# skyplane-project/skyplane

Measured on NVIDIA H100. Metric: chunk-pipeline GB/s (raw input), higher is better.
Workload: dtype u8/u32

## Files before the change

skyplane_b200/csrc/md5.cuh:

```cuda
#pragma once
#include <stdint.h>

#include <type_traits>
#include <utility>

#ifndef SKY_MD5_SLOTS
#define SKY_MD5_SLOTS 4
#endif

namespace sky {

struct Md5State {
    uint32_t a, b, c, d;
};

__device__ __forceinline__ void md5_init(Md5State &s) {
    s.a = 0x67452301u;
    s.b = 0xefcdab89u;
    s.c = 0x98badcfeu;
    s.d = 0x10325476u;
}

__device__ __forceinline__ uint32_t md5_am(uint32_t a, uint32_t m, uint32_t one) {
    uint32_t r;
    asm("mad.lo.u32 %0, %1, %2, %3;" : "=r"(r) : "r"(m), "r"(one), "r"(a));
    return r;
}
__device__ __forceinline__ uint32_t md5_one() {
    uint32_t eq, lane;
    asm("mov.u32 %0, %%lanemask_eq;" : "=r"(eq));
    asm("mov.u32 %0, %%laneid;" : "=r"(lane));
    return eq >> lane;
}
#define SKY_MD5_STEP(FN, a, b, c, d, m, k, s)                      \
    {                                                              \
        uint32_t t_ = FN(b, c, d) + md5_am(a, (m), one) + (k);     \
        a = b + __funnelshift_l(t_, t_, s);                        \
    }
#define SKY_F(b, c, d) ((d) ^ ((b) & ((c) ^ (d))))
#define SKY_G(b, c, d) ((c) ^ ((d) & ((b) ^ (c))))
#define SKY_H(b, c, d) ((b) ^ (c) ^ (d))
#define SKY_I(b, c, d) ((c) ^ ((b) | ~(d)))

template <int R>
__device__ __forceinline__ void md5_round(uint32_t &a, uint32_t &b, uint32_t &c, uint32_t &d, const uint32_t (&w)[16],
                                          uint32_t one) {
    if constexpr (R == 0) {
        SKY_MD5_STEP(SKY_F, a, b, c, d, w[0], 0xd76aa478, 7)
        SKY_MD5_STEP(SKY_F, d, a, b, c, w[1], 0xe8c7b756, 12)
        SKY_MD5_STEP(SKY_F, c, d, a, b, w[2], 0x242070db, 17)
        SKY_MD5_STEP(SKY_F, b, c, d, a, w[3], 0xc1bdceee, 22)
        SKY_MD5_STEP(SKY_F, a, b, c, d, w[4], 0xf57c0faf, 7)
        SKY_MD5_STEP(SKY_F, d, a, b, c, w[5], 0x4787c62a, 12)
        SKY_MD5_STEP(SKY_F, c, d, a, b, w[6], 0xa8304613, 17)
        SKY_MD5_STEP(SKY_F, b, c, d, a, w[7], 0xfd469501, 22)
        SKY_MD5_STEP(SKY_F, a, b, c, d, w[8], 0x698098d8, 7)
        SKY_MD5_STEP(SKY_F, d, a, b, c, w[9], 0x8b44f7af, 12)
        SKY_MD5_STEP(SKY_F, c, d, a, b, w[10], 0xffff5bb1, 17)
        SKY_MD5_STEP(SKY_F, b, c, d, a, w[11], 0x895cd7be, 22)
        SKY_MD5_STEP(SKY_F, a, b, c, d, w[12], 0x6b901122, 7)
        SKY_MD5_STEP(SKY_F, d, a, b, c, w[13], 0xfd987193, 12)
        SKY_MD5_STEP(SKY_F, c, d, a, b, w[14], 0xa679438e, 17)
        SKY_MD5_STEP(SKY_F, b, c, d, a, w[15], 0x49b40821, 22)
    } else if constexpr (R == 1) {
        SKY_MD5_STEP(SKY_G, a, b, c, d, w[1], 0xf61e2562, 5)
        SKY_MD5_STEP(SKY_G, d, a, b, c, w[6], 0xc040b340, 9)
        SKY_MD5_STEP(SKY_G, c, d, a, b, w[11], 0x265e5a51, 14)
        SKY_MD5_STEP(SKY_G, b, c, d, a, w[0], 0xe9b6c7aa, 20)
        SKY_MD5_STEP(SKY_G, a, b, c, d, w[5], 0xd62f105d, 5)
        SKY_MD5_STEP(SKY_G, d, a, b, c, w[10], 0x02441453, 9)
        SKY_MD5_STEP(SKY_G, c, d, a, b, w[15], 0xd8a1e681, 14)
        SKY_MD5_STEP(SKY_G, b, c, d, a, w[4], 0xe7d3fbc8, 20)
        SKY_MD5_STEP(SKY_G, a, b, c, d, w[9], 0x21e1cde6, 5)
        SKY_MD5_STEP(SKY_G, d, a, b, c, w[14], 0xc33707d6, 9)
        SKY_MD5_STEP(SKY_G, c, d, a, b, w[3], 0xf4d50d87, 14)
        SKY_MD5_STEP(SKY_G, b, c, d, a, w[8], 0x455a14ed, 20)
        SKY_MD5_STEP(SKY_G, a, b, c, d, w[13], 0xa9e3e905, 5)
        SKY_MD5_STEP(SKY_G, d, a, b, c, w[2], 0xfcefa3f8, 9)
        SKY_MD5_STEP(SKY_G, c, d, a, b, w[7], 0x676f02d9, 14)
        SKY_MD5_STEP(SKY_G, b, c, d, a, w[12], 0x8d2a4c8a, 20)
    } else if constexpr (R == 2) {
        SKY_MD5_STEP(SKY_H, a, b, c, d, w[5], 0xfffa3942, 4)
        SKY_MD5_STEP(SKY_H, d, a, b, c, w[8], 0x8771f681, 11)
        SKY_MD5_STEP(SKY_H, c, d, a, b, w[11], 0x6d9d6122, 16)
        SKY_MD5_STEP(SKY_H, b, c, d, a, w[14], 0xfde5380c, 23)
        SKY_MD5_STEP(SKY_H, a, b, c, d, w[1], 0xa4beea44, 4)
        SKY_MD5_STEP(SKY_H, d, a, b, c, w[4], 0x4bdecfa9, 11)
        SKY_MD5_STEP(SKY_H, c, d, a, b, w[7], 0xf6bb4b60, 16)
        SKY_MD5_STEP(SKY_H, b, c, d, a, w[10], 0xbebfbc70, 23)
        SKY_MD5_STEP(SKY_H, a, b, c, d, w[13], 0x289b7ec6, 4)
        SKY_MD5_STEP(SKY_H, d, a, b, c, w[0], 0xeaa127fa, 11)
        SKY_MD5_STEP(SKY_H, c, d, a, b, w[3], 0xd4ef3085, 16)
        SKY_MD5_STEP(SKY_H, b, c, d, a, w[6], 0x04881d05, 23)
        SKY_MD5_STEP(SKY_H, a, b, c, d, w[9], 0xd9d4d039, 4)
        SKY_MD5_STEP(SKY_H, d, a, b, c, w[12], 0xe6db99e5, 11)
        SKY_MD5_STEP(SKY_H, c, d, a, b, w[15], 0x1fa27cf8, 16)
        SKY_MD5_STEP(SKY_H, b, c, d, a, w[2], 0xc4ac5665, 23)
    } else {
        SKY_MD5_STEP(SKY_I, a, b, c, d, w[0], 0xf4292244, 6)
        SKY_MD5_STEP(SKY_I, d, a, b, c, w[7], 0x432aff97, 10)
        SKY_MD5_STEP(SKY_I, c, d, a, b, w[14], 0xab9423a7, 15)
        SKY_MD5_STEP(SKY_I, b, c, d, a, w[5], 0xfc93a039, 21)
        SKY_MD5_STEP(SKY_I, a, b, c, d, w[12], 0x655b59c3, 6)
        SKY_MD5_STEP(SKY_I, d, a, b, c, w[3], 0x8f0ccc92, 10)
        SKY_MD5_STEP(SKY_I, c, d, a, b, w[10], 0xffeff47d, 15)
        SKY_MD5_STEP(SKY_I, b, c, d, a, w[1], 0x85845dd1, 21)
        SKY_MD5_STEP(SKY_I, a, b, c, d, w[8], 0x6fa87e4f, 6)
        SKY_MD5_STEP(SKY_I, d, a, b, c, w[15], 0xfe2ce6e0, 10)
        SKY_MD5_STEP(SKY_I, c, d, a, b, w[6], 0xa3014314, 15)
        SKY_MD5_STEP(SKY_I, b, c, d, a, w[13], 0x4e0811a1, 21)
        SKY_MD5_STEP(SKY_I, a, b, c, d, w[4], 0xf7537e82, 6)
        SKY_MD5_STEP(SKY_I, d, a, b, c, w[11], 0xbd3af235, 10)
        SKY_MD5_STEP(SKY_I, c, d, a, b, w[2], 0x2ad7d2bb, 15)
        SKY_MD5_STEP(SKY_I, b, c, d, a, w[9], 0xeb86d391, 21)
    }
}

__device__ __forceinline__ void md5_block(Md5State &st, const uint32_t (&w)[16], uint32_t one) {
    uint32_t a = st.a, b = st.b, c = st.c, d = st.d;
    md5_round<0>(a, b, c, d, w, one);
    md5_round<1>(a, b, c, d, w, one);
    md5_round<2>(a, b, c, d, w, one);
    md5_round<3>(a, b, c, d, w, one);
    st.a += a;
    st.b += b;
    st.c += c;
    st.d += d;
}

template <int kSlot>
__device__ __forceinline__ void cp_async_block(bool pred, uint32_t lane_ring, const uint8_t *gptr) {
    asm volatile(
        "{\n\t.reg .pred p;\n\t"
        "setp.ne.b32 p, %2, 0;\n\t"
        "@p cp.async.cg.shared.global [%0+%3], [%1], 16;\n\t"
        "@p cp.async.cg.shared.global [%0+%4], [%1+16], 16;\n\t"
        "@p cp.async.cg.shared.global [%0+%5], [%1+32], 16;\n\t"
        "@p cp.async.cg.shared.global [%0+%6], [%1+48], 16;\n\t}" ::"r"(lane_ring),
        "l"(gptr), "r"((uint32_t)pred), "n"(kSlot * 2048), "n"(kSlot * 2048 + 512), "n"(kSlot * 2048 + 1024),
        "n"(kSlot * 2048 + 1536)
        : "memory");
}
__device__ __forceinline__ void cp_async_commit() { asm volatile("cp.async.commit_group;\n" ::: "memory"); }
template <int N>
__device__ __forceinline__ void cp_async_wait() {
    asm volatile("cp.async.wait_group %0;\n" ::"n"(N) : "memory");
}

template <class F, int... I>
__device__ __forceinline__ void md5_unroll_(F &&f, std::integer_sequence<int, I...>) {
    (f(std::integral_constant<int, I>()), ...);
}
template <int N, class F>
__device__ __forceinline__ void md5_unroll(F &&f) {
    md5_unroll_(f, std::make_integer_sequence<int, N>());
}

struct Md5NoGate {
    __device__ __forceinline__ void operator()(uint64_t, bool) const {}
};

template <class Gate = Md5NoGate>
__device__ __forceinline__ void md5_warp(uint32_t *ring, const uint8_t *src, uint64_t len, bool active, uint8_t *out,
                                         unsigned lane, Gate gate = Gate()) {
    constexpr int kSlots = SKY_MD5_SLOTS;
    static_assert(kSlots >= 2 && (kSlots & (kSlots - 1)) == 0 && 1024 % kSlots == 0, "SKY_MD5_SLOTS: a power of two, 2..1024");
    constexpr bool kGated = !std::is_same<Gate, Md5NoGate>::value;
    const uint32_t nfull = active ? (uint32_t)(len >> 6) : 0;
    const uint32_t wmax = __reduce_max_sync(0xffffffffu, nfull);
    const uint32_t trips = (wmax + (kSlots - 1)) & ~(uint32_t)(kSlots - 1);
    Md5State st;
    md5_init(st);
    Md5State fin = st;
    const uint32_t *lring = ring + lane * 4;
    const uint32_t lring_s = (uint32_t)__cvta_generic_to_shared(lring);
    const uint32_t one = md5_one();

    gate(0, active && len > 0);
    md5_unroll<kSlots - 1>([&](auto sc) {
        constexpr int s = decltype(sc)::value;
        cp_async_block<s>((uint32_t)s < nfull, lring_s, src + s * 64);
        cp_async_commit();
    });
    auto load_words = [&](uint32_t (&w)[16], int cs) {
#pragma unroll
        for (int q = 0; q < 4; q++) {
            const uint4 v = *reinterpret_cast<const uint4 *>(lring + (cs * 4 + q) * 128);
            w[4 * q + 0] = v.x;
            w[4 * q + 1] = v.y;
            w[4 * q + 2] = v.z;
            w[4 * q + 3] = v.w;
        }
    };
    uint32_t w[2][16];
    cp_async_wait<kSlots - 2>();
    load_words(w[0], 0);
    const uint8_t *pf_src = src + (kSlots - 1) * 64;
    auto blocks = [&](uint32_t i) {
        md5_unroll<kSlots>([&](auto uc) {
            constexpr int u = decltype(uc)::value;
            constexpr int ps = (u + kSlots - 1) & (kSlots - 1);
            constexpr int ns = (u + 1) & (kSlots - 1);
            uint32_t a = st.a, b = st.b, c = st.c, d = st.d;
            md5_round<0>(a, b, c, d, w[u & 1], one);
            cp_async_block<ps>(i + u + (kSlots - 1) < nfull, lring_s, pf_src + u * 64);
            md5_round<1>(a, b, c, d, w[u & 1], one);
            cp_async_commit();
            cp_async_wait<kSlots - 2>();
            md5_round<2>(a, b, c, d, w[u & 1], one);
            load_words(w[(u + 1) & 1], ns);
            md5_round<3>(a, b, c, d, w[u & 1], one);
            st.a += a;
            st.b += b;
            st.c += c;
            st.d += d;
            if (i + u < nfull) fin = st;
        });
        pf_src += kSlots * 64;
    };
    if constexpr (kGated) {
        for (uint32_t base = 0; base < trips; base += 1024) {
            gate((base >> 10) + 1, (uint64_t)(base + 1024) * 64 < len);
            const uint32_t iend = min(base + 1024, trips);
            for (uint32_t i = base; i < iend; i += kSlots) blocks(i);
        }
    } else {
        for (uint32_t i = 0; i < trips; i += kSlots) blocks(i);
    }
    cp_async_wait<0>();
    st = fin;
    if (active) {
        const uint32_t rem = (uint32_t)(len & 63);
        const uint8_t *tp = src + ((uint64_t)nfull << 6);
        uint32_t tw[32];
#pragma unroll
        for (int k = 0; k < 32; k++) tw[k] = 0;
        for (uint32_t k = 0; k < rem; k++) tw[k >> 2] |= (uint32_t)tp[k] << (8 * (k & 3));
        tw[rem >> 2] |= 0x80u << (8 * (rem & 3));
        const bool two = rem >= 56;
        const uint64_t bits = len << 3;
        tw[two ? 30 : 14] = (uint32_t)bits;
        tw[two ? 31 : 15] = (uint32_t)(bits >> 32);
        for (int t = 0; t < (two ? 2 : 1); t++) {
            uint32_t w[16];
#pragma unroll
            for (int k = 0; k < 16; k++) w[k] = tw[16 * t + k];
            md5_block(st, w, one);
        }
        uint4 dg = make_uint4(st.a, st.b, st.c, st.d);
        *reinterpret_cast<uint4 *>(out) = dg;
    }
}

}
```

skyplane_b200/native.py:

```python
from __future__ import annotations

import ctypes
from pathlib import Path
from typing import Optional, Sequence

_PKG = Path(__file__).resolve().parent
LIB_PATH = _PKG / "libskychunk.so"

SKY_OK = 0
SKY_E_INVALID, SKY_E_NOGPU, SKY_E_CUDA, SKY_E_CAPACITY, SKY_E_BUSY, SKY_E_TICKET, SKY_E_NOMEM, SKY_E_NOKEY = -1, -2, -3, -4, -5, -6, -7, -8
F_LZ4, F_MD5, F_E2EE, F_HC = 1, 2, 16, 32
BOX_OVERHEAD = 40
D_OK, D_BAD_HEADER, D_CORRUPT, D_SIZE, D_UNSUPPORTED, D_LAYOUT, D_TRUNCATED, D_AUTH = 0, -1, -2, -3, -4, -5, -6, -7
D_NAMES = {0: "ok", -1: "bad frame header", -2: "corrupt block", -3: "size mismatch", -4: "unsupported frame feature",
           -5: "unexpected block layout", -6: "truncated frame", -7: "box authentication failed"}

ABI_SYMBOLS = (
    "sky_strerror", "sky_last_error", "sky_abi_version", "sky_device_count", "sky_device_pci_bus_id", "sky_kernel_config", "sky_frame_bound",
    "sky_ctx_create", "sky_ctx_destroy", "sky_pinned_alloc", "sky_pinned_free",
    "sky_submit", "sky_wait", "sky_set_e2ee_key", "sky_box_bound", "sky_process_device", "sky_decode_device", "sky_decode",
    "sky_device_alloc", "sky_device_free", "sky_memcpy_h2d", "sky_memcpy_d2h", "sky_launch_count",
)


class SkyChunkError(RuntimeError):
    def __init__(self, code: int, detail: str = ""):
        self.code = code
        msg = f"libskychunk error {code}: {_strerror(code)}"
        if detail:
            msg += f" [{detail}]"
        super().__init__(msg)


_lib: Optional[ctypes.CDLL] = None


def _strerror(code: int) -> str:
    try:
        return lib().sky_strerror(code).decode()
    except Exception:
        return "?"


def lib() -> ctypes.CDLL:
    global _lib
    if _lib is not None:
        return _lib
    import os

    from skyplane_b200 import build as _build

    override = os.environ.get("SKYCHUNK_LIB")
    if override:
        L = ctypes.CDLL(override)
    else:
        if _build.needs_build():
            _build.build()
        L = ctypes.CDLL(str(LIB_PATH))
    vp, u64, u32, i32 = ctypes.c_void_p, ctypes.c_uint64, ctypes.c_uint32, ctypes.c_int
    p_u64 = ctypes.POINTER(u64)
    L.sky_strerror.argtypes = [i32]
    L.sky_strerror.restype = ctypes.c_char_p
    L.sky_last_error.argtypes = [vp]
    L.sky_last_error.restype = ctypes.c_char_p
    L.sky_abi_version.argtypes = []
    L.sky_abi_version.restype = i32
    L.sky_device_count.argtypes = [ctypes.POINTER(i32)]
    L.sky_device_count.restype = i32
    L.sky_device_pci_bus_id.argtypes = [i32, ctypes.c_char_p, i32]
    L.sky_device_pci_bus_id.restype = i32
    L.sky_kernel_config.argtypes = [i32]
    L.sky_kernel_config.restype = u32
    L.sky_frame_bound.argtypes = [u64]
    L.sky_frame_bound.restype = u64
    L.sky_ctx_create.argtypes = [i32, u64, u32, u32, ctypes.POINTER(vp)]
    L.sky_ctx_create.restype = i32
    L.sky_ctx_destroy.argtypes = [vp]
    L.sky_ctx_destroy.restype = i32
    L.sky_pinned_alloc.argtypes = [u64]
    L.sky_pinned_alloc.restype = vp
    L.sky_pinned_free.argtypes = [vp]
    L.sky_pinned_free.restype = i32
    L.sky_submit.argtypes = [vp, u32, ctypes.POINTER(vp), p_u64, ctypes.POINTER(vp), p_u64, u32, ctypes.c_char_p, p_u64]
    L.sky_submit.restype = i32
    L.sky_set_e2ee_key.argtypes = [vp, ctypes.c_char_p]
    L.sky_set_e2ee_key.restype = i32
    L.sky_box_bound.argtypes = [u64]
    L.sky_box_bound.restype = u64
    L.sky_wait.argtypes = [vp, u64, p_u64, vp, ctypes.POINTER(ctypes.c_float)]
    L.sky_wait.restype = i32
    L.sky_process_device.argtypes = [vp, u32, vp, p_u64, p_u64, vp, p_u64, p_u64, u32, vp, p_u64, vp, ctypes.POINTER(ctypes.c_float)]
    L.sky_process_device.restype = i32
    p_i32 = ctypes.POINTER(ctypes.c_int32)
    L.sky_decode_device.argtypes = [vp, u32, vp, p_u64, p_u64, vp, p_u64, p_u64, vp, p_i32, vp, ctypes.POINTER(ctypes.c_float)]
    L.sky_decode_device.restype = i32
    L.sky_decode.argtypes = [vp, u32, ctypes.POINTER(vp), p_u64, ctypes.POINTER(vp), p_u64, u32, p_i32, vp, ctypes.POINTER(ctypes.c_float)]
    L.sky_decode.restype = i32
    L.sky_device_alloc.argtypes = [vp, u64, ctypes.POINTER(vp)]
    L.sky_device_alloc.restype = i32
    L.sky_device_free.argtypes = [vp, vp]
    L.sky_device_free.restype = i32
    L.sky_memcpy_h2d.argtypes = [vp, vp, vp, u64]
    L.sky_memcpy_h2d.restype = i32
    L.sky_memcpy_d2h.argtypes = [vp, vp, vp, u64]
    L.sky_memcpy_d2h.restype = i32
    L.sky_launch_count.argtypes = [vp]
    L.sky_launch_count.restype = u64
    _lib = L
    return L


def device_pci_bus_id(device: int) -> str:
    buf = ctypes.create_string_buffer(32)
    rc = lib().sky_device_pci_bus_id(device, buf, 32)
    if rc != SKY_OK:
        raise SkyChunkError(rc)
    return buf.value.decode().lower()


def kernel_config() -> dict:
    L = lib()
    return {"lz4_entries": L.sky_kernel_config(0), "warps": L.sky_kernel_config(1), "seg_slots": L.sky_kernel_config(2),
            "max_step_log": L.sky_kernel_config(3), "hc_depth": L.sky_kernel_config(4), "hc_hash_bits": L.sky_kernel_config(5),
            "hc_nice": L.sky_kernel_config(6)}


def frame_bound(n: int) -> int:
    return int(lib().sky_frame_bound(n))


def round16(x: int) -> int:
    return (x + 15) & ~15


def device_count() -> int:
    n = ctypes.c_int(0)
    rc = lib().sky_device_count(ctypes.byref(n))
    if rc != SKY_OK:
        return 0
    return n.value


class PinnedBuffer:

    def __init__(self, nbytes: int):
        self.nbytes = int(nbytes)
        self.addr = lib().sky_pinned_alloc(self.nbytes)
        if not self.addr:
            raise SkyChunkError(SKY_E_NOMEM, "sky_pinned_alloc failed (no CUDA device?)")
        self._arr = (ctypes.c_ubyte * max(1, self.nbytes)).from_address(self.addr)
        self.view = memoryview(self._arr).cast("B")[: self.nbytes]

    def close(self):
        if self.addr:
            self.view.release()
            del self._arr
            lib().sky_pinned_free(self.addr)
            self.addr = None

    def __del__(self):
        try:
            self.close()
        except Exception:
            pass


class Context:

    def __init__(self, device: int = 0, max_batch_bytes: int = 1 << 30, max_chunks: int = 1024, n_slots: int = 2):
        self._h = ctypes.c_void_p()
        self.device = device
        self.max_chunks = max_chunks
        self.max_batch_bytes = max_batch_bytes
        rc = lib().sky_ctx_create(device, max_batch_bytes, max_chunks, n_slots, ctypes.byref(self._h))
        if rc != SKY_OK:
            detail = lib().sky_last_error(None).decode()
            self._h = ctypes.c_void_p()
            raise SkyChunkError(rc, detail)
        self._inflight = {}

    def _check(self, rc: int):
        if rc != SKY_OK:
            raise SkyChunkError(rc, lib().sky_last_error(self._h).decode())

    def close(self):
        if self._h:
            lib().sky_ctx_destroy(self._h)
            self._h = ctypes.c_void_p()

    def __enter__(self):
        return self

    def __exit__(self, *exc):
        self.close()

    def __del__(self):
        try:
            self.close()
        except Exception:
            pass

    @property
    def launches(self) -> int:
        return int(lib().sky_launch_count(self._h))

    def set_e2ee_key(self, key: Optional[bytes]):
        if key is not None and len(key) != 32:
            raise ValueError("SecretBox keys are 32 bytes")
        self._check(lib().sky_set_e2ee_key(self._h, key))

    def submit(self, src_addrs: Sequence[int], src_lens: Sequence[int], dst_addrs: Optional[Sequence[int]], dst_caps: Optional[Sequence[int]],
               flags: int = 0, nonces: Optional[bytes] = None) -> int:
        n = len(src_addrs)
        A = ctypes.c_void_p * n
        U = ctypes.c_uint64 * n
        args = (A(*src_addrs), U(*src_lens), A(*dst_addrs) if dst_addrs is not None else None, U(*dst_caps) if dst_caps is not None else None, nonces)
        if nonces is not None and len(nonces) != 24 * n:
            raise ValueError("need 24 nonce bytes per chunk")
        t = ctypes.c_uint64(0)
        self._check(lib().sky_submit(self._h, n, args[0], args[1], args[2], args[3], flags, nonces, ctypes.byref(t)))
        self._inflight[t.value] = (n, args)
        return t.value

    def wait(self, ticket: int):
        n, _keep = self._inflight.pop(ticket)
        out = (ctypes.c_uint64 * n)()
        md5 = (ctypes.c_ubyte * (16 * n))()
        ms = ctypes.c_float(0)
        self._check(lib().sky_wait(self._h, ticket, out, md5, ctypes.byref(ms)))
        raw = bytes(md5)
        return list(out), [raw[16 * i : 16 * i + 16] for i in range(n)], ms.value

    def process_device(self, d_src: int, src_off: Sequence[int], src_len: Sequence[int], d_dst: int, dst_off: Sequence[int],
                       dst_cap: Sequence[int], flags: int = 0, stream: int = 0):
        n = len(src_len)
        U = ctypes.c_uint64 * n
        out = U()
        md5 = (ctypes.c_ubyte * (16 * n))()
        ms = ctypes.c_float(0)
        self._check(
            lib().sky_process_device(self._h, n, d_src, U(*src_off), U(*src_len), d_dst, U(*dst_off), U(*dst_cap), flags,
                                     stream or None, out, md5, ctypes.byref(ms))
        )
        raw = bytes(md5)
        return list(out), [raw[16 * i : 16 * i + 16] for i in range(n)], ms.value

    def decode_device(self, d_frames: int, frame_off: Sequence[int], frame_len: Sequence[int], d_out: int, out_off: Sequence[int],
                      raw_len: Sequence[int], stream: int = 0):
        n = len(frame_len)
        U = ctypes.c_uint64 * n
        st = (ctypes.c_int32 * n)()
        md5 = (ctypes.c_ubyte * (16 * n))()
        ms = ctypes.c_float(0)
        self._check(lib().sky_decode_device(self._h, n, d_frames, U(*frame_off), U(*frame_len), d_out, U(*out_off), U(*raw_len),
                                            stream or None, st, md5, ctypes.byref(ms)))
        raw = bytes(md5)
        return list(st), [raw[16 * i : 16 * i + 16] for i in range(n)], ms.value

    def decode(self, frame_addrs: Sequence[int], frame_lens: Sequence[int], dst_addrs: Sequence[int], raw_lens: Sequence[int], flags: int = 0):
        n = len(frame_addrs)
        A = ctypes.c_void_p * n
        U = ctypes.c_uint64 * n
        st = (ctypes.c_int32 * n)()
        md5 = (ctypes.c_ubyte * (16 * n))()
        ms = ctypes.c_float(0)
        self._check(lib().sky_decode(self._h, n, A(*frame_addrs), U(*frame_lens), A(*dst_addrs), U(*raw_lens), flags, st, md5, ctypes.byref(ms)))
        raw = bytes(md5)
        return list(st), [raw[16 * i : 16 * i + 16] for i in range(n)], ms.value

    def device_alloc(self, nbytes: int) -> int:
        p = ctypes.c_void_p()
        self._check(lib().sky_device_alloc(self._h, nbytes, ctypes.byref(p)))
        return p.value

    def device_free(self, dptr: int):
        self._check(lib().sky_device_free(self._h, dptr))

    def h2d(self, dptr: int, data) -> None:
        mv = memoryview(data).cast("B")
        if mv.nbytes == 0:
            return
        buf = (ctypes.c_ubyte * mv.nbytes).from_buffer_copy(mv) if mv.readonly else (ctypes.c_ubyte * mv.nbytes).from_buffer(mv)
        self._check(lib().sky_memcpy_h2d(self._h, dptr, ctypes.addressof(buf), mv.nbytes))

    def d2h(self, dptr: int, nbytes: int) -> bytes:
        if nbytes == 0:
            return b""
        buf = (ctypes.c_ubyte * nbytes)()
        self._check(lib().sky_memcpy_d2h(self._h, ctypes.addressof(buf), dptr, nbytes))
        return bytes(buf)
```

Baseline: 157.6.

## Add L2 128B prefetch hint to cp.async and speed up Python argument marshalling

The MD5 staging loads now carry the L2::128B prefetch qualifier, so each 16-byte async copy asks L2 to fetch the whole 128-byte sector line and later lane loads hit it. Separately, the Python wrapper builds uint64 argument arrays through array.array buffers instead of ctypes star-unpacking, and splits digests with struct.unpack. Both aim to cut per-call overhead: global-memory latency in the kernel and ctypes marshalling on the host. The prefetch hint may waste bandwidth when the access pattern already covers full lines.

```diff
diff --git a/skyplane_b200/csrc/md5.cuh b/skyplane_b200/csrc/md5.cuh
--- a/skyplane_b200/csrc/md5.cuh
+++ b/skyplane_b200/csrc/md5.cuh
@@ -133,10 +133,10 @@
     asm volatile(
         "{\n\t.reg .pred p;\n\t"
         "setp.ne.b32 p, %2, 0;\n\t"
-        "@p cp.async.cg.shared.global [%0+%3], [%1], 16;\n\t"
-        "@p cp.async.cg.shared.global [%0+%4], [%1+16], 16;\n\t"
-        "@p cp.async.cg.shared.global [%0+%5], [%1+32], 16;\n\t"
-        "@p cp.async.cg.shared.global [%0+%6], [%1+48], 16;\n\t}" ::"r"(lane_ring),
+        "@p cp.async.cg.shared.global.L2::128B [%0+%3], [%1], 16;\n\t"
+        "@p cp.async.cg.shared.global.L2::128B [%0+%4], [%1+16], 16;\n\t"
+        "@p cp.async.cg.shared.global.L2::128B [%0+%5], [%1+32], 16;\n\t"
+        "@p cp.async.cg.shared.global.L2::128B [%0+%6], [%1+48], 16;\n\t}" ::"r"(lane_ring),
         "l"(gptr), "r"((uint32_t)pred), "n"(kSlot * 2048), "n"(kSlot * 2048 + 512), "n"(kSlot * 2048 + 1024),
         "n"(kSlot * 2048 + 1536)
         : "memory");
diff --git a/skyplane_b200/native.py b/skyplane_b200/native.py
--- a/skyplane_b200/native.py
+++ b/skyplane_b200/native.py
@@ -1,6 +1,8 @@
 from __future__ import annotations
 
+import array
 import ctypes
+import struct
 from pathlib import Path
 from typing import Optional, Sequence
 
@@ -141,6 +143,15 @@
     return n.value
 
 
+def _u64(seq) -> ctypes.Array:
+    a = seq if isinstance(seq, array.array) and seq.typecode == "Q" else array.array("Q", seq)
+    return (ctypes.c_uint64 * len(a)).from_buffer(a)
+
+
+def _digests(md5, n: int) -> list:
+    return list(struct.unpack("16s" * n, md5))
+
+
 class PinnedBuffer:
 
     def __init__(self, nbytes: int):
@@ -228,22 +239,19 @@
         md5 = (ctypes.c_ubyte * (16 * n))()
         ms = ctypes.c_float(0)
         self._check(lib().sky_wait(self._h, ticket, out, md5, ctypes.byref(ms)))
-        raw = bytes(md5)
-        return list(out), [raw[16 * i : 16 * i + 16] for i in range(n)], ms.value
+        return list(out), _digests(md5, n), ms.value
 
     def process_device(self, d_src: int, src_off: Sequence[int], src_len: Sequence[int], d_dst: int, dst_off: Sequence[int],
                        dst_cap: Sequence[int], flags: int = 0, stream: int = 0):
         n = len(src_len)
-        U = ctypes.c_uint64 * n
-        out = U()
+        out = array.array("Q", bytes(8 * n))
         md5 = (ctypes.c_ubyte * (16 * n))()
         ms = ctypes.c_float(0)
         self._check(
-            lib().sky_process_device(self._h, n, d_src, U(*src_off), U(*src_len), d_dst, U(*dst_off), U(*dst_cap), flags,
-                                     stream or None, out, md5, ctypes.byref(ms))
+            lib().sky_process_device(self._h, n, d_src, _u64(src_off), _u64(src_len), d_dst, _u64(dst_off), _u64(dst_cap), flags,
+                                     stream or None, _u64(out), md5, ctypes.byref(ms))
         )
-        raw = bytes(md5)
-        return list(out), [raw[16 * i : 16 * i + 16] for i in range(n)], ms.value
+        return out.tolist(), _digests(md5, n), ms.value
 
     def decode_device(self, d_frames: int, frame_off: Sequence[int], frame_len: Sequence[int], d_out: int, out_off: Sequence[int],
                       raw_len: Sequence[int], stream: int = 0):
@@ -254,8 +262,7 @@
         ms = ctypes.c_float(0)
         self._check(lib().sky_decode_device(self._h, n, d_frames, U(*frame_off), U(*frame_len), d_out, U(*out_off), U(*raw_len),
                                             stream or None, st, md5, ctypes.byref(ms)))
-        raw = bytes(md5)
-        return list(st), [raw[16 * i : 16 * i + 16] for i in range(n)], ms.value
+        return list(st), _digests(md5, n), ms.value
 
     def decode(self, frame_addrs: Sequence[int], frame_lens: Sequence[int], dst_addrs: Sequence[int], raw_lens: Sequence[int], flags: int = 0):
         n = len(frame_addrs)
@@ -265,8 +272,7 @@
         md5 = (ctypes.c_ubyte * (16 * n))()
         ms = ctypes.c_float(0)
         self._check(lib().sky_decode(self._h, n, A(*frame_addrs), U(*frame_lens), A(*dst_addrs), U(*raw_lens), flags, st, md5, ctypes.byref(ms)))
-        raw = bytes(md5)
-        return list(st), [raw[16 * i : 16 * i + 16] for i in range(n)], ms.value
+        return list(st), _digests(md5, n), ms.value
 
     def device_alloc(self, nbytes: int) -> int:
         p = ctypes.c_void_p()
```

Measured after the change: 160.7, median of 6. 1.02x the previous value.
